# Siyou-Li/u2Tokenizer

Measured on AMD Instinct MI355X. Metric: CT volumes/sec (256^3 fp16) through u2Tokenizer fwd, higher is better.
Workload: dtype bf16; 1 GPU; BASELINE configs[2]: u2Qwen3-8B-shaped path, 256^3 volume = 8x(32,256,256) fp16, ViT-B 3D x12, SPP, 4-layer rma+diffts+dmtp tokenizer (8 heads, top_k 1024, scales {1,2,4}, 256 queries), text 1024, prompt 1024; hidden_size=4096, batch_per_gpu=1, streams_per_gpu=2, parallelism=replicas x1, tta_side_stream=off in the multi-stream run, on in the one-stream run

## Files before the change

### include/u2tok.h

```cpp
#ifndef U2TOK_H_
#define U2TOK_H_

#include <stddef.h>
#include <stdint.h>

#ifdef __cplusplus
extern "C" {
#endif

#define U2TOK_OK 0
#define U2TOK_ERR_ARG (-1)
#define U2TOK_ERR_LAUNCH (-2)
#define U2TOK_ERR_WORKSPACE (-3)
#define U2TOK_ERR_DEVICE (-4)

typedef void* u2tok_stream_t;

int u2tok_version(void);
const char* u2tok_arch(void);
const char* u2tok_elem(void);
int u2tok_device_check(void);
typedef struct u2tok_ctx* u2tok_ctx_t;
int u2tok_ctx_create(u2tok_ctx_t* out);
int u2tok_ctx_destroy(u2tok_ctx_t ctx);
int u2tok_ctx_set_current(u2tok_ctx_t ctx);
u2tok_ctx_t u2tok_ctx_get_current(void);

int u2tok_set_option(const char* name, int value);
int u2tok_set_gemm_scratch(void* device_ptr, size_t bytes, void* stream);

int u2tok_profile_collect(double* ms_host, double* flops_host, int64_t* count_host, int32_t ncat);
int u2tok_profile_collect2(double* ms_host, double* flops_host, double* bytes_host, int64_t* count_host, int32_t ncat);


typedef struct {
  int32_t nchunk;
  int32_t img[3];
  int32_t patch[3];
  int32_t hidden;
  int32_t mlp_dim;
  int32_t depth;
  int32_t heads;
  int32_t vol_dtype;
// ... 48 lines not shown
int u2tok_tokenizer_forward(const u2tok_tokenizer_config* cfg, const void* const* weights, const void* v_token,
                            const void* t_token, void* out, int64_t* topk_idx_out, void* svr_out, void* workspace,
                            size_t workspace_bytes, u2tok_stream_t stream);

typedef struct {
  const void* const* svr_in;
  void* const* svr_out;
  const void* visual_in;
  void* visual_out;
  const void* const* tta_in;
  void* const* tta_out;
} u2tok_tokenizer_taps;
int u2tok_tokenizer_forward_taps(const u2tok_tokenizer_config* cfg, const void* const* weights, const void* v_token,
                                 const void* t_token, void* out, int64_t* topk_idx_out, const u2tok_tokenizer_taps* taps,
                                 void* workspace, size_t workspace_bytes, u2tok_stream_t stream);

int u2tok_embed_splice(const void* table, const int64_t* ids, const void* feats, void* out, int32_t B, int32_t S,
                       int32_t E, int32_t nfeat, int64_t vocab, u2tok_stream_t stream);

size_t u2tok_preprocess_workspace_bytes(int32_t D, int32_t H, int32_t W);
int u2tok_preprocess_volume(const float* vol, void* out, int32_t* info, int32_t D, int32_t H, int32_t W, int32_t target,
                            int32_t depth_pad, float lower_pct, float upper_pct, int32_t out_dtype, void* workspace,
                            size_t workspace_bytes, u2tok_stream_t stream);

typedef struct {
  int32_t rot90_k;
  int32_t flip[3];
  float scale_factor;
  float shift_offset;
} u2tok_augment;
// ... 169 lines not shown
```

### u2tokenizer_amd/_lib.py

```python
from __future__ import annotations

import ctypes as C
import os
import subprocess
import threading
from pathlib import Path

_PKG = Path(__file__).resolve().parent
_LIB = _PKG / "lib" / "libu2tok_hip.so"
_LIBS = {"bf16": _LIB, "f16": _PKG / "lib" / "libu2tok_hip_f16.so"}
_lock = threading.Lock()
_handles = {}


class LibraryNotBuilt(RuntimeError):
    pass


def lib_path() -> Path:
    return _LIB


def build(verbose: bool = False) -> Path:
    cmd = ["make", "-C", str(_PKG / "csrc"), "-j", str(os.cpu_count() or 4)]
# ... 39 lines not shown
    _fields_ = [("rot90_k", C.c_int32), ("flip", C.c_int32 * 3), ("scale_factor", C.c_float), ("shift_offset", C.c_float)]


_vp, _i32, _i64, _f32, _sz = C.c_void_p, C.c_int32, C.c_int64, C.c_float, C.c_size_t

SIGNATURES = {
    "u2tok_version": (_i32, []),
    "u2tok_arch": (C.c_char_p, []),
    "u2tok_elem": (C.c_char_p, []),
    "u2tok_device_check": (_i32, []),
    "u2tok_ctx_create": (_i32, [C.POINTER(_vp)]),
    "u2tok_ctx_destroy": (_i32, [_vp]),
    "u2tok_ctx_set_current": (_i32, [_vp]),
    "u2tok_ctx_get_current": (_vp, []),
    "u2tok_set_option": (_i32, [C.c_char_p, _i32]),
    "u2tok_profile_collect": (_i32, [_vp, _vp, _vp, _i32]),
    "u2tok_profile_collect2": (_i32, [_vp, _vp, _vp, _vp, _i32]),
    "u2tok_set_gemm_scratch": (_i32, [_vp, _sz, _vp]),
    "u2tok_vit_workspace_bytes": (_sz, [C.POINTER(VitConfig)]),
    "u2tok_vit_forward": (_i32, [C.POINTER(VitConfig), C.POINTER(_vp), _vp, _vp, _vp, _sz, _vp]),
    "u2tok_spp_workspace_bytes": (_sz, [C.POINTER(SppConfig)]),
    "u2tok_spp_forward": (_i32, [C.POINTER(SppConfig), C.POINTER(_vp), _vp, _vp, _vp, _sz, _vp]),
    "u2tok_tokenizer_workspace_bytes": (_sz, [C.POINTER(TokConfig)]),
    "u2tok_tokenizer_forward": (_i32, [C.POINTER(TokConfig), C.POINTER(_vp), _vp, _vp, _vp, _vp, _vp, _vp, _sz, _vp]),
    "u2tok_tokenizer_forward_taps": (_i32, [C.POINTER(TokConfig), C.POINTER(_vp), _vp, _vp, _vp, _vp, C.POINTER(TokTaps),
                                            _vp, _sz, _vp]),
    "u2tok_tok_attention_workspace_bytes": (_sz, [_i32, _i32, _i32, _i32, _i32]),
    "u2tok_tok_attention": (_i32, [_vp, _vp, _vp, _vp, _i32, _i32, _i32, _i32, _i32, _i64, _i64, _i64, _i64, _i64, _i64, _i64,
                                   _i64, _f32, _vp, _i32, _i32, _vp, _sz, _vp]),
    "u2tok_preprocess_workspace_bytes": (_sz, [_i32, _i32, _i32]),
    "u2tok_preprocess_volume": (_i32, [_vp, _vp, _vp, _i32, _i32, _i32, _i32, _i32, _f32, _f32, _i32, _vp, _sz, _vp]),
    "u2tok_preprocess_volume_aug": (_i32, [_vp, _vp, _vp, _i32, _i32, _i32, _i32, _i32, _f32, _f32, _i32,
                                           C.POINTER(Augment), _vp, _sz, _vp]),
    "u2tok_embed_splice": (_i32, [_vp, _vp, _vp, _vp, _i32, _i32, _i32, _i32, _i64, _vp]),
    "u2tok_gemm_bf16": (_i32, [_vp, _vp, _vp, _vp, _vp, _i32, _i32, _i32, _i64, _i64, _i64, _i64, _i32, _i32,
                               _i64, _i64, _i64, _i64, _i64, _i64, _i64, _i64, _f32, _i32, _vp]),
    "u2tok_layernorm_bf16": (_i32, [_vp, _vp, _vp, _vp, _vp, _i32, _i32, _f32, _vp]),
    "u2tok_softmax_rows": (_i32, [_vp, _vp, _i32, _i32, _i32, _i64, _i64, _f32, _vp, _i32, _i32, _vp]),
    "u2tok_transpose_bf16": (_i32, [_vp, _vp, _i32, _i32, _i32, _i64, _i64, _i64, _i64, _i32, _vp]),
    "u2tok_im2col_patches": (_i32, [_vp, _i32, _vp, _i32, _i32, _i32, _i32, _i32, _i32, _i32, _vp]),
    "u2tok_avgpool3d_tokens": (_i32, [_vp, _vp, _i32, _i32, _i32, _i32, _i32, _i32, _i32, _i32, _vp]),
# ... 117 lines not shown
```

### u2tokenizer_amd/csrc/capi.hip

```cpp
#include <math.h>
#include <string.h>
#include <new>
#include "pipeline.h"

using namespace u2;

static_assert(U2TOK_OK == U2_OK && U2TOK_ERR_ARG == U2_ERR_ARG && U2TOK_ERR_LAUNCH == U2_ERR_LAUNCH &&
                  U2TOK_ERR_WORKSPACE == U2_ERR_WORKSPACE && U2TOK_ERR_DEVICE == U2_ERR_DEVICE,
              "public and internal status codes must agree");

#define BF(p) reinterpret_cast<const bf16_t*>(p)
#define BFW(p) reinterpret_cast<bf16_t*>(p)
#define ST(s) reinterpret_cast<hipStream_t>(s)

extern "C" {

int u2tok_version(void) { return 100;  }
const char* u2tok_arch(void) { return "gfx950"; }
const char* u2tok_elem(void) { return U2_ELEM_ASM; }

int u2tok_device_check(void) {
  int dev = 0;
  if (hipGetDevice(&dev) != hipSuccess) return U2_ERR_DEVICE;
  hipDeviceProp_t prop;
// ... 7 lines not shown
  return *out ? U2_OK : U2_ERR_ARG;
}
int u2tok_ctx_destroy(u2tok_ctx_t c) {
  if (!c) return U2_ERR_ARG;
  Context* cx = reinterpret_cast<Context*>(c);
  if (ctx_bound() == cx) ctx_bind(nullptr);
  delete cx;
  return U2_OK;
}
int u2tok_ctx_set_current(u2tok_ctx_t c) {
  ctx_bind(reinterpret_cast<Context*>(c));
  return U2_OK;
}
u2tok_ctx_t u2tok_ctx_get_current(void) { return reinterpret_cast<u2tok_ctx_t>(ctx_bound()); }

int u2tok_set_option(const char* name, int value) {
  if (!name) return U2_ERR_ARG;
  Options& o = ctx().opt;
  struct Opt { const char* name; int Options::*field; int lo, hi; };
  static const Opt table[] = {
      {"gemm_splitk", &Options::gemm_splitk, -1, 16},   {"gemm_mubuf", &Options::gemm_mubuf, 0, 1}, {"ln_wide", &Options::ln_wide, 0, 1},   {"gemm_big", &Options::gemm_big, -1, 27},
      {"gemm_big_grid", &Options::gemm_big_grid, 1, 4096}, {"gemm_big_splitk", &Options::gemm_big_splitk, 0, 16},
      {"gemm_big_drain", &Options::gemm_big_drain, 0, 1}, {"gemm_skinny", &Options::gemm_skinny, 0, 2},
       {"kmajor_b", &Options::kmajor_b, 0, 1},            {"gemm_tail_fused", &Options::gemm_tail_fused, 0, 1},
      {"flash_mode", &Options::flash_mode, 0, 7},        {"flash_q_prescaled", &Options::flash_q_prescaled, 0, 1},
      {"vit_flash", &Options::vit_flash, 0, 1},         {"tta_overlap", &Options::tta_overlap, 0, 1},
      {"vit_vt_epilogue", &Options::vit_vt_epilogue, 0, 1},
      {"tok_flash", &Options::tok_flash, 0, 1},
      {"tok_wide", &Options::tok_wide, 0, 2},
  };
  if (!strcmp(name, "gemm_tile")) {
    if (value != 0 && value != 64 && value != 128) return U2_ERR_ARG;
    o.gemm_tile = value;
    return U2_OK;
  }
  if (!strcmp(name, "profile")) { prof_enable(value != 0); return U2_OK; }
  for (const Opt& t : table)
    if (!strcmp(name, t.name)) {
      if (value < t.lo || value > t.hi) return U2_ERR_ARG;
      if (t.field == &Options::gemm_big && value > 0 && !(value >= 20 && value <= 27 && value != 23 && value != 25)) return U2_ERR_ARG;
      if (t.field == &Options::flash_mode && value != 0 && value != 1 && value != 7) return U2_ERR_ARG;
      o.*(t.field) = value;
      return U2_OK;
    }
  return U2_ERR_ARG;
}

int u2tok_set_gemm_scratch(void* device_ptr, size_t bytes, void* stream) {
  ctx().set_scratch(reinterpret_cast<hipStream_t>(stream), device_ptr, device_ptr ? bytes : 0);
  return U2_OK;
}

int u2tok_profile_collect(double* ms, double* flops, int64_t* count, int32_t ncat) {
  if (!ms || !flops || !count || ncat <= 0 || ncat > PROF_NCAT) return U2_ERR_ARG;
  return prof_collect(ms, flops, nullptr, count, ncat);
}
int u2tok_profile_collect2(double* ms, double* flops, double* bytes, int64_t* count, int32_t ncat) {
  if (!ms || !flops || !bytes || !count || ncat <= 0 || ncat > PROF_NCAT) return U2_ERR_ARG;
  return prof_collect(ms, flops, bytes, count, ncat);
}

// ... 30 lines not shown
  return peak + 256;
}
int u2tok_tokenizer_forward(const u2tok_tokenizer_config* cfg, const void* const* weights, const void* v_token,
                            const void* t_token, void* out, int64_t* topk_idx_out, void* svr_out, void* workspace,
                            size_t workspace_bytes, u2tok_stream_t stream) {
  if (!cfg || !workspace || ((uintptr_t)workspace & 255)) return U2_ERR_ARG;
  return tokenizer_forward(*cfg, weights, BF(v_token), BF(t_token), BFW(out), topk_idx_out, BFW(svr_out), nullptr, workspace,
                           workspace_bytes, false, nullptr, ST(stream));
}
int u2tok_tokenizer_forward_taps(const u2tok_tokenizer_config* cfg, const void* const* weights, const void* v_token,
                                 const void* t_token, void* out, int64_t* topk_idx_out, const u2tok_tokenizer_taps* taps,
                                 void* workspace, size_t workspace_bytes, u2tok_stream_t stream) {
  if (!cfg || !taps || !workspace || ((uintptr_t)workspace & 255)) return U2_ERR_ARG;
  return tokenizer_forward(*cfg, weights, BF(v_token), BF(t_token), BFW(out), topk_idx_out, nullptr, taps, workspace,
                           workspace_bytes, false, nullptr, ST(stream));
}

size_t u2tok_preprocess_workspace_bytes(int32_t D, int32_t H, int32_t W) { return preprocess_workspace_bytes(D, H, W); }
int u2tok_preprocess_volume(const float* vol, void* out, int32_t* info, int32_t D, int32_t H, int32_t W, int32_t target,
                            int32_t depth_pad, float lower_pct, float upper_pct, int32_t out_dtype, void* workspace,
                            size_t workspace_bytes, u2tok_stream_t stream) {
  return preprocess_volume(vol, out, info, D, H, W, target, depth_pad, lower_pct, upper_pct, out_dtype, nullptr, workspace,
                           workspace_bytes, ST(stream));
}
int u2tok_preprocess_volume_aug(const float* vol, void* out, int32_t* info, int32_t D, int32_t H, int32_t W, int32_t target,
                                int32_t depth_pad, float lower_pct, float upper_pct, int32_t out_dtype,
                                const u2tok_augment* aug, void* workspace, size_t workspace_bytes, u2tok_stream_t stream) {
  if (!aug) return U2_ERR_ARG;
  PreAugment a;
  a.rot_k = aug->rot90_k;
// ... 355 lines not shown
```

### u2tokenizer_amd/csrc/ctx.h

```cpp
#pragma once
#include <mutex>
#include <vector>
#include "common.h"

namespace u2 {

struct Options {
  int ln_wide = 1;
  int gemm_tile = 0;
  int gemm_mubuf = 1;
  int gemm_splitk = 0;
  int gemm_big = 0;
  int gemm_big_grid = 256;
  int gemm_big_splitk = 0;
  int gemm_big_drain = 1;
  int gemm_skinny = 2;
  int gemm_tail_fused = 1;
  int kmajor_b = 1;
  int flash_mode = 0;
  int flash_q_prescaled = 0;
  int vit_flash = 1;
  int vit_vt_epilogue = 1;
  int tok_flash = 1;
  int tok_wide = 2;
  int tta_overlap = 1;
  int profile = 0;
};

struct SideStream {
  hipStream_t owner = nullptr;
  hipStream_t s = nullptr;
  hipEvent_t fork = nullptr;
  hipEvent_t done[16] = {};
};

struct Scratch {
  hipStream_t st;
  void* p;
  size_t bytes;
};

struct ProfRec {
  hipEvent_t a, b;
  int cat;
  double flops, bytes;
};

struct Context {
  Options opt;
  std::mutex mu;
  std::vector<SideStream*> sides;
  std::vector<Scratch> scratch;
  std::vector<ProfRec> recs;
  std::vector<hipEvent_t> ev_pool;
  size_t ev_used = 0;

  SideStream* side_for(hipStream_t owner);
  void set_scratch(hipStream_t st, void* p, size_t bytes);
  Scratch scratch_of(hipStream_t st);
  void release();
  ~Context() { release(); }
};

Context& ctx();
// ... 6 lines not shown
```

### u2tokenizer_amd/csrc/pipeline.h

```cpp
#pragma once
#include <algorithm>
#include "../../include/u2tok.h"
#include "kernels.h"

namespace u2 {

typedef u2tok_vit_config VitConfig;
typedef u2tok_spp_config SppConfig;
typedef u2tok_tokenizer_config TokConfig;
typedef u2tok_tokenizer_taps TokTaps;

int vit_forward(const VitConfig& c, const void* const* W, const void* volume, bf16_t* out, void* ws, size_t ws_bytes,
                bool dry, size_t* peak, hipStream_t st);
int spp_forward(const SppConfig& c, const void* const* W, const bf16_t* x, bf16_t* out, void* ws, size_t ws_bytes,
                bool dry, size_t* peak, hipStream_t st);
int tokenizer_forward(const TokConfig& c, const void* const* W, const bf16_t* v_token, const bf16_t* t_token,
                      bf16_t* out, int64_t* topk_idx_out, bf16_t* svr_out, const TokTaps* taps, void* ws, size_t ws_bytes,
                      bool dry, size_t* peak, hipStream_t st);

}
```

### u2tokenizer_amd/csrc/pipeline.hip

```cpp
#include "pipeline.h"

namespace u2 {

namespace {

struct Arena {
  char* base;
  size_t cap;
  size_t off = 0, peak = 0;
  bool dry;
  Arena(void* b, size_t c, bool d) : base((char*)b), cap(c), dry(d) {}
  template <typename T>
  T* get(size_t count) {
    const size_t a = (off + 255) & ~(size_t)255;
    off = a + count * sizeof(T);
    if (off > peak) peak = off;
    if (dry) return reinterpret_cast<T*>((uintptr_t)0x1000 + a);
    return (off <= cap) ? reinterpret_cast<T*>(base + a) : nullptr;
  }
  bool ok() const { return dry || peak <= cap; }
};

struct ScratchScope {
  Context& cx;
// ... 275 lines not shown
  return a.wk && a.bk && a.wv == a.wk + (size_t)E * E && a.bv == a.bk + E;
}
inline bool qkv_packed(const Att& a, int E) {
  return a.wq && a.bq && a.wk == a.wq + (size_t)E * E && a.bk == a.bq + E && kv_packed(a, E);
}
int qkv_proj(const bf16_t* x, const Att& a, bf16_t* out, int64_t rows, int E, bool dry, hipStream_t st) {
  if (!dry && qkv_packed(a, E)) {
    U2_RUN(linear(x, E, a.wq, a.bq, out, 3 * E, rows, E, 3 * E, 0, nullptr, 0, st));
    return U2_OK;
  }
  U2_RUN(linear(x, E, a.wq, a.bq, out, 3 * E, rows, E, E, 0, nullptr, 0, st));
  U2_RUN(linear(x, E, a.wk, a.bk, out + E, 3 * E, rows, E, E, 0, nullptr, 0, st));
  U2_RUN(linear(x, E, a.wv, a.bv, out + 2 * E, 3 * E, rows, E, E, 0, nullptr, 0, st));
  return U2_OK;
}
}

int tokenizer_forward(const TokConfig& c, const void* const* W, const bf16_t* v_token, const bf16_t* t_token,
                      bf16_t* out, int64_t* topk_idx_out, bf16_t* svr_out, const TokTaps* taps, void* ws, size_t ws_bytes,
                      bool dry, size_t* peak, hipStream_t st) {
  if (c.B <= 0 || c.T <= 0 || c.N <= 0 || c.E <= 0 || c.Lt <= 0 || c.num_heads <= 0 || c.num_layers < 0) return U2_ERR_ARG;
  if (c.E % c.num_heads || (c.E / c.num_heads) % 8 || c.top_k <= 0 || c.num_query <= 0) return U2_ERR_ARG;
  if (c.attn_type < 0 || c.attn_type > 2) return U2_ERR_ARG;
  if (!dry && (!W || !v_token || !t_token || !out)) return U2_ERR_ARG;
  const int B = c.B, T = c.T, N = c.N, E = c.E, H = c.num_heads, d = E / H, L = c.num_layers, Q = c.num_query;
  const int TN = T * N, k = c.top_k;
  if (!c.enable_diffts && k > TN) return U2_ERR_ARG;
  if (N > c.max_seq_len || T > c.max_seq_len || Q > c.max_seq_len) return U2_ERR_ARG;
  const float scale = 1.0f / sqrtf((float)d);
  auto wp = [&](int i) { return dry ? nullptr : reinterpret_cast<const bf16_t*>(W[i]); };
  auto att_at = [&](int i) {
    Att a{wp(i), wp(i + 1), wp(i + 2), wp(i + 3), wp(i + 4), wp(i + 5), wp(i + 6), wp(i + 7), wp(i + 8)};
    if (c.attn_type != 0) a.rb = nullptr;
    return a;
  };
  const int i_sel = 1 + 18 * L, i_gate = i_sel + 2, i_tta = i_gate + 2, i_lin = i_tta + 33 * L;

  Arena ar(ws, ws_bytes, dry);
  const size_t kSplitK = std::max<size_t>(24u << 20, (size_t)16 * B * c.num_query * 3 * E);
  char* skw = ar.get<char>(kSplitK);
  U2_CHECK_WS(ar);
  Context& cx = ctx();
  ScratchScope scratch_scope(cx, st, skw, kSplitK, !dry);
  const int64_t rows = (int64_t)B * TN;
  bf16_t* xa = ar.get<bf16_t>((size_t)rows * E);
  bf16_t* xb = ar.get<bf16_t>((size_t)rows * E);
  bf16_t* qkv = ar.get<bf16_t>((size_t)rows * 3 * E);
  bf16_t* ctx = ar.get<bf16_t>((size_t)rows * E);
  U2_CHECK_WS(ar);

  const bf16_t* x = v_token;
  for (int l = 0; l < L; ++l) {
    const Att sp = att_at(1 + 18 * l), tp = att_at(1 + 18 * l + 9);
    if (taps && !dry && taps->svr_in && taps->svr_in[l]) x = reinterpret_cast<const bf16_t*>(taps->svr_in[l]);
// ... 157 lines not shown
  if (overlap && !dry) {
    if (hipEventRecord(side->fork, st) != hipSuccess || hipStreamWaitEvent(side->s, side->fork, 0) != hipSuccess)
      return U2_ERR_LAUNCH;
    for (int l = 0; l < L; ++l) {
      const int base = i_tta + 33 * l;
      Att va = att_at(base + 9), ta = att_at(base + 18);
      { const int e = kv_proj(va, V, Lv, kv_v[l], side->s); if (e != U2_OK) return e; }
      if (hipEventRecord(side->done[2 * l], side->s) != hipSuccess) return U2_ERR_LAUNCH;
      { const int e = kv_proj(ta, t_token, c.Lt, kv_t[l], side->s); if (e != U2_OK) return e; }
      if (hipEventRecord(side->done[2 * l + 1], side->s) != hipSuccess) return U2_ERR_LAUNCH;
    }
    const Att la = att_at(i_lin);
    U2_RUN(linear(V, E, la.wk, la.bk, k_lin, E, (int64_t)B * Lv, E, E, 0, nullptr, 0, side->s));
    if (hipEventRecord(side->done[2 * L], side->s) != hipSuccess) return U2_ERR_LAUNCH;
  }
  U2_RUN(fill_rows(wp(0), qa, B, (int64_t)Q * E, (int64_t)Q * E, st));
  bf16_t* qcur = qa;
  auto cross = [&](const Att& a, const bf16_t* src, int Ls, const bf16_t* qin, bf16_t* dst, bf16_t* kv,
                   int kv_ready) -> int {
    U2_RUN(linear(qin, E, a.wq, a.bq, qproj, E, qrows, E, E, 0, nullptr, 0, st));
    if (kv_ready < 0) {
      const int e = kv_proj(a, src, Ls, kv, st);
      if (e != U2_OK) return e;
    } else if (!dry) {
      if (hipStreamWaitEvent(st, side->done[kv_ready], 0) != hipSuccess) return U2_ERR_LAUNCH;
    }
    AttnCore ac{qproj, kv, kv + E, E, 2 * E, 2 * E, (int64_t)Q * E, (int64_t)Ls * 2 * E, (int64_t)Ls * 2 * E,
                qctx, E, (int64_t)Q * E, B, Q, Ls, H, d, scale, nullptr, 0};
    const int e = attention_core(ar, ac, dry, st);
    if (e != U2_OK) return e;
    U2_RUN(linear(qctx, E, a.wd, a.bd, dst, E, qrows, E, E, 0, nullptr, 0, st));
    return U2_OK;
  };
  for (int l = 0; l < L; ++l) {
    const int base = i_tta + 33 * l;
    const Att sa = att_at(base);
    Att va = att_at(base + 9), ta = att_at(base + 18);
    va.rb = ta.rb = nullptr;
    const bf16_t *ns_w = wp(base + 27), *ns_b = wp(base + 28), *nv_w = wp(base + 29), *nv_b = wp(base + 30),
                 *nt_w = wp(base + 31), *nt_b = wp(base + 32);
    if (taps && !dry && taps->tta_in && taps->tta_in[l]) qcur = (bf16_t*)taps->tta_in[l];
    bf16_t* s1 = (qcur == qa) ? qb : qa;
    bf16_t* s2 = qc;
    if (c.attn_type == 2 && B == 1) {
      U2_RUN(linear(qcur, E, sa.wv, sa.bv, qctx, E, qrows, E, E, 0, nullptr, 0, st));
    } else if (c.attn_type == 2) {
      { const int e = qkv_proj(qcur, sa, qproj, qrows, E, dry, st); if (e != U2_OK) return e; }
      const int e = chunk_axis_attention(ar, qproj, qctx, 1, B, Q, H, d, scale, nullptr, c.max_seq_len, dry, st);
      if (e != U2_OK) return e;
    } else {
      { const int e = qkv_proj(qcur, sa, qproj, qrows, E, dry, st); if (e != U2_OK) return e; }
      if (c.attn_type == 1) {
        U2_RUN(rope_apply(qproj, B, Q, 1, H, d, 3 * E, c.max_seq_len, 0, st));
        U2_RUN(rope_apply(qproj + E, B, Q, 1, H, d, 3 * E, c.max_seq_len, 0, st));
      }
      AttnCore ac{qproj, qproj + E, qproj + 2 * E, 3 * E, 3 * E, 3 * E, (int64_t)Q * 3 * E, (int64_t)Q * 3 * E,
                  (int64_t)Q * 3 * E, qctx, E, (int64_t)Q * E, B, Q, Q, H, d, scale, sa.rb, c.max_seq_len};
      const int e = attention_core(ar, ac, dry, st);
      if (e != U2_OK) return e;
    }
    U2_RUN(linear(qctx, E, sa.wd, sa.bd, qo, E, qrows, E, E, 0, nullptr, 0, st));
    U2_RUN(layernorm_bf16(qcur, qo, ns_w, ns_b, s1, 1, (int)qrows, E, 0, E, 0, E, 0, E, c.ln_eps, st));
    { const int e = cross(va, V, Lv, s1, qo, overlap ? kv_v[l] : kv_inline, overlap ? 2 * l : -1); if (e != U2_OK) return e; }
    U2_RUN(layernorm_bf16(s1, qo, nv_w, nv_b, s2, 1, (int)qrows, E, 0, E, 0, E, 0, E, c.ln_eps, st));
    { const int e = cross(ta, t_token, c.Lt, s2, qo, overlap ? kv_t[l] : kv_inline, overlap ? 2 * l + 1 : -1); if (e != U2_OK) return e; }
    U2_RUN(layernorm_bf16(s2, qo, nt_w, nt_b, s1, 1, (int)qrows, E, 0, E, 0, E, 0, E, c.ln_eps, st));
    qcur = s1;
    if (taps && !dry && taps->tta_out && taps->tta_out[l] &&
        hipMemcpyAsync(taps->tta_out[l], qcur, (size_t)qrows * E * sizeof(bf16_t), hipMemcpyDeviceToDevice, st) != hipSuccess)
      return U2_ERR_LAUNCH;
  }
  {
    const Att la = att_at(i_lin);
    U2_RUN(linear(qcur, E, la.wq, la.bq, qproj, E, qrows, E, E, 0, nullptr, 0, st));
    if (!overlap) {
      U2_RUN(linear(V, E, la.wk, la.bk, k_lin, E, (int64_t)B * Lv, E, E, 0, nullptr, 0, st));
    } else if (!dry) {
      if (hipStreamWaitEvent(st, side->done[2 * L], 0) != hipSuccess) return U2_ERR_LAUNCH;
    }
    AttnCore ac{qproj, k_lin, V, E, E, E, (int64_t)Q * E, (int64_t)Lv * E, (int64_t)Lv * E,
                out, E, (int64_t)Q * E, B, Q, Lv, H, d, scale, nullptr, 0};
    const int e = attention_core(ar, ac, dry, st);
// ... 9 lines not shown
```

### u2tokenizer_amd/tokenizer.py

```python
from __future__ import annotations

import ctypes as C

import torch
import torch.nn as nn

from . import _lib, ops

_ATTN_TYPES = {"rma": 0, "rope": 1}


def _init_attn(m):
    for lin in (m.wq, m.wk, m.wv, m.dense):
        nn.init.xavier_uniform_(lin.weight)
        if lin.bias is not None:
            nn.init.zeros_(lin.bias)


class RelativeMultiheadAttention(nn.Module):

    def __init__(self, d_model, num_heads, max_seq_len=512):
        super().__init__()
        assert d_model % num_heads == 0
        self.num_heads, self.d_model, self.depth, self.max_seq_len = num_heads, d_model, d_model // num_heads, max_seq_len
# ... 176 lines not shown
        if embed_size != hidden_size:
            raise ValueError("embed_size must equal hidden_size (builder.py:5,11 pass config.hidden_size for both)")
        self.svt_module = SpatioTemporalVisualTokenRefinerModel(
            embed_size=embed_size, num_heads=num_heads, num_layers=num_layers, top_k=top_k,
            use_multi_scale=use_multi_scale, attn_type=attn_type, enable_diffts=enable_diffts,
            enable_dmtp=enable_dmtp)
        self.tta_module = TextConditionTokenAggregatorModel(d_model=embed_size, num_layers=num_layers,
                                                            num_heads=num_heads, attn_type=attn_type)
        self.query_tokens = nn.Parameter(torch.zeros(1, num_3d_query_token, hidden_size))
        self.query_tokens.data.normal_(mean=0.0, std=0.02)
        self.embed_size, self.num_heads, self.num_layers, self.top_k = embed_size, num_heads, num_layers, top_k
        self.use_multi_scale, self.num_query, self.attn_type = bool(use_multi_scale), num_3d_query_token, attn_type
        self.enable_diffts, self.enable_dmtp = bool(enable_diffts), bool(enable_dmtp)
        self._ws = ops._Workspace()
        self._packed_key = None
        self._dead_offloaded = False
        self._register_state_dict_hook(_unshare_packed)
        self.last_topk_indices = None
        self.capture_svr_tokens = False
        self.last_svr_tokens = None

    def _weights(self):
        w = [self.query_tokens]
        for layer in self.svt_module.attention_network.layers:
            w += _att_ptrs(layer.spatial_attention) + _att_ptrs(layer.temporal_attention)
        sn = self.svt_module.token_selection.score_net
        w += [sn.weight, sn.bias]
        if self.enable_dmtp:
            w += [self.svt_module.dynamic_pool.gate_fc.weight, self.svt_module.dynamic_pool.gate_fc.bias]
        else:
# ... 10 lines not shown
        key = (self.query_tokens.data_ptr(), self.query_tokens.dtype)
        if self._packed_key == key:
            return
        with torch.no_grad():
            for layer in self.svt_module.attention_network.layers:
                _pack_qkv(layer.spatial_attention)
                _pack_qkv(layer.temporal_attention)
            for layer in self.tta_module.layers_vt:
                for m in (layer.self_attention, layer.visual_cross_attention, layer.text_cross_attention):
                    _pack_qkv(m)
        if self.query_tokens.is_cuda:
            torch.cuda.synchronize(self.query_tokens.device)
        self._packed_key = key

    def _apply(self, fn, *args, **kwargs):
        r = super()._apply(fn, *args, **kwargs)
        self._packed_key = None
        if self.query_tokens.is_cuda:
            self.pack_weights()
            if self._dead_offloaded:
                self.offload_dead_parameters()
        return r

    def dead_parameters(self):
        la = self.tta_module.layer_linagg.linear_aggregator
        return [la.wv.weight, la.wv.bias, la.dense.weight, la.dense.bias]

    def offload_dead_parameters(self) -> int:
        freed = 0
        for p in self.dead_parameters():
            if p.is_cuda:
                freed += p.numel() * p.element_size()
                p.data = p.data.to("cpu")
            p.requires_grad_(False)
        self._dead_offloaded = True
        return freed

# ... 40 lines not shown
            return arr

        svr_out = [torch.empty((B, T, N, E), dtype=ops.elem_dtype(), device=dev) for _ in range(L)]
        tta_out = [torch.empty((B, Q, E), dtype=ops.elem_dtype(), device=dev) for _ in range(L)]
        visual_out = torch.empty((B, Lv, E), dtype=ops.elem_dtype(), device=dev)
        if visual_in is not None:
            visual_in = ops._need(visual_in, ops.ELEM, "visual_in").contiguous()
            assert tuple(visual_in.shape) == (B, Lv, E)
        taps = _lib.TokTaps(svr_in=ptr_array(svr_in, (B, T, N, E)), svr_out=ptr_array(svr_out, (B, T, N, E)),
                            visual_in=None if visual_in is None else visual_in.data_ptr(), visual_out=visual_out.data_ptr(),
                            tta_in=ptr_array(tta_in, (B, Q, E)), tta_out=ptr_array(tta_out, (B, Q, E)))
        with ops.on_device(v_token) as (h, stream):
            ws = self._ws.get(nbytes, dev)
            out = torch.empty((B, Q, E), dtype=ops.elem_dtype(), device=dev)
            idx = None if self.enable_diffts else torch.empty((B, self.top_k), dtype=torch.int64, device=dev)
            _lib.check(h.u2tok_tokenizer_forward_taps(C.byref(cfg), table, v_token.data_ptr(), t_token.data_ptr(),
                                                      out.data_ptr(), None if idx is None else idx.data_ptr(),
                                                      C.byref(taps), ws.data_ptr(), ws.numel(), stream),
                       "u2tok_tokenizer_forward_taps")
        self.last_topk_indices = idx
        return out, {"svr_out": svr_out, "visual_out": visual_out, "tta_out": tta_out}

    def _config(self, B, T, N, E, Lt):
        return _lib.TokConfig(B=B, T=T, N=N, E=E, Lt=Lt, num_heads=self.num_heads,
                              num_layers=self.num_layers, top_k=self.top_k, num_query=self.num_query,
                              use_multi_scale=int(self.use_multi_scale), attn_type=_ATTN_TYPES.get(self.attn_type, 2),
                              enable_diffts=int(self.enable_diffts), enable_dmtp=int(self.enable_dmtp),
                              max_seq_len=512, diffts_tau=float(getattr(self.svt_module.token_selection, "tau", 1.0)),
                              ln_eps=1e-5)

    def forward(self, v_token, t_token):
        with ops.on_device(v_token, elem=self.query_tokens.dtype):
            return self._forward(v_token, t_token)

# ... 18 lines not shown
        self._check_envelope(B, T, N, E, t_token.shape[1])
        cfg = self._config(B, T, N, E, t_token.shape[1])
        table = ops.weight_table(self._weights())
        nbytes = h.u2tok_tokenizer_workspace_bytes(C.byref(cfg))
        if nbytes == 0:
            raise RuntimeError("u2tok_tokenizer_workspace_bytes rejected the configuration "
                               f"(B={B}, T={T}, N={N}, E={E}, heads={self.num_heads}, top_k={self.top_k})")
        idx = svr = None
        with ops.on_device(v_token) as (h, stream):
            ws = self._ws.get(nbytes, v_token.device)
            out = torch.empty((B, self.num_query, E), dtype=ops.elem_dtype(), device=v_token.device)
            if not self.enable_diffts:
                idx = torch.empty((B, self.top_k), dtype=torch.int64, device=v_token.device)
            if self.capture_svr_tokens:
                svr = torch.empty((B, T * N, E), dtype=ops.elem_dtype(), device=v_token.device)
            _lib.check(h.u2tok_tokenizer_forward(C.byref(cfg), table, v_token.data_ptr(), t_token.data_ptr(),
                                                 out.data_ptr(), None if idx is None else idx.data_ptr(),
                                                 None if svr is None else svr.data_ptr(), ws.data_ptr(), ws.numel(),
                                                 stream), "u2tok_tokenizer_forward")
        self.last_topk_indices = idx
        self.last_svr_tokens = svr
        return out
```

Measured before the change: 128.2 volumes/s.

## Precompute and cache weight-only first TTA layer query prefix across forwards

Adds a C API that computes, from weights alone, the first TTA layer's query self-attention, norm and visual-query projection. It also adds a prefixed forward entry that consumes these results in place of recomputing them. The Python tokenizer caches the prefix per batch size and invalidates it on weight version, pointer, option-epoch or context change. This removes a few small per-call GEMMs and an attention at the cost of cache management, host synchronisation when the prefix is rebuilt, and extra option plumbing.

```diff
diff --git a/include/u2tok.h b/include/u2tok.h
--- a/include/u2tok.h
+++ b/include/u2tok.h
@@ -27,6 +27,8 @@
 u2tok_ctx_t u2tok_ctx_get_current(void);
 
 int u2tok_set_option(const char* name, int value);
+int u2tok_get_option(const char* name, int* value);
+int64_t u2tok_option_epoch(void);
 int u2tok_set_gemm_scratch(void* device_ptr, size_t bytes, void* stream);
 
 int u2tok_profile_collect(double* ms_host, double* flops_host, int64_t* count_host, int32_t ncat);
@@ -105,6 +107,13 @@
 int u2tok_tokenizer_forward_taps(const u2tok_tokenizer_config* cfg, const void* const* weights, const void* v_token,
                                  const void* t_token, void* out, int64_t* topk_idx_out, const u2tok_tokenizer_taps* taps,
                                  void* workspace, size_t workspace_bytes, u2tok_stream_t stream);
+
+int u2tok_tokenizer_query_prefix(const u2tok_tokenizer_config* cfg, const void* const* weights, void* s1_out, void* q_out,
+                                 void* workspace, size_t workspace_bytes, u2tok_stream_t stream);
+int u2tok_tokenizer_forward_prefixed(const u2tok_tokenizer_config* cfg, const void* const* weights, const void* v_token,
+                                     const void* t_token, void* out, int64_t* topk_idx_out, void* svr_out,
+                                     const u2tok_tokenizer_taps* taps, const void* prefix_s1, const void* prefix_q,
+                                     void* workspace, size_t workspace_bytes, u2tok_stream_t stream);
 
 int u2tok_embed_splice(const void* table, const int64_t* ids, const void* feats, void* out, int32_t B, int32_t S,
                        int32_t E, int32_t nfeat, int64_t vocab, u2tok_stream_t stream);
diff --git a/u2tokenizer_amd/_lib.py b/u2tokenizer_amd/_lib.py
--- a/u2tokenizer_amd/_lib.py
+++ b/u2tokenizer_amd/_lib.py
@@ -77,6 +77,8 @@
     "u2tok_ctx_set_current": (_i32, [_vp]),
     "u2tok_ctx_get_current": (_vp, []),
     "u2tok_set_option": (_i32, [C.c_char_p, _i32]),
+    "u2tok_get_option": (_i32, [C.c_char_p, C.POINTER(_i32)]),
+    "u2tok_option_epoch": (_i64, []),
     "u2tok_profile_collect": (_i32, [_vp, _vp, _vp, _i32]),
     "u2tok_profile_collect2": (_i32, [_vp, _vp, _vp, _vp, _i32]),
     "u2tok_set_gemm_scratch": (_i32, [_vp, _sz, _vp]),
@@ -88,6 +90,9 @@
     "u2tok_tokenizer_forward": (_i32, [C.POINTER(TokConfig), C.POINTER(_vp), _vp, _vp, _vp, _vp, _vp, _vp, _sz, _vp]),
     "u2tok_tokenizer_forward_taps": (_i32, [C.POINTER(TokConfig), C.POINTER(_vp), _vp, _vp, _vp, _vp, C.POINTER(TokTaps),
                                             _vp, _sz, _vp]),
+    "u2tok_tokenizer_query_prefix": (_i32, [C.POINTER(TokConfig), C.POINTER(_vp), _vp, _vp, _vp, _sz, _vp]),
+    "u2tok_tokenizer_forward_prefixed": (_i32, [C.POINTER(TokConfig), C.POINTER(_vp), _vp, _vp, _vp, _vp, _vp,
+                                                C.POINTER(TokTaps), _vp, _vp, _vp, _sz, _vp]),
     "u2tok_tok_attention_workspace_bytes": (_sz, [_i32, _i32, _i32, _i32, _i32]),
     "u2tok_tok_attention": (_i32, [_vp, _vp, _vp, _vp, _i32, _i32, _i32, _i32, _i32, _i64, _i64, _i64, _i64, _i64, _i64, _i64,
                                    _i64, _f32, _vp, _i32, _i32, _vp, _sz, _vp]),
diff --git a/u2tokenizer_amd/csrc/capi.hip b/u2tokenizer_amd/csrc/capi.hip
--- a/u2tokenizer_amd/csrc/capi.hip
+++ b/u2tokenizer_amd/csrc/capi.hip
@@ -45,37 +45,51 @@
 }
 u2tok_ctx_t u2tok_ctx_get_current(void) { return reinterpret_cast<u2tok_ctx_t>(ctx_bound()); }
 
+namespace {
+struct Opt { const char* name; int Options::*field; int lo, hi; };
+const Opt kOptions[] = {
+    {"gemm_splitk", &Options::gemm_splitk, -1, 16},   {"gemm_mubuf", &Options::gemm_mubuf, 0, 1}, {"ln_wide", &Options::ln_wide, 0, 1},   {"gemm_big", &Options::gemm_big, -1, 27},
+    {"gemm_big_grid", &Options::gemm_big_grid, 1, 4096}, {"gemm_big_splitk", &Options::gemm_big_splitk, 0, 16},
+    {"gemm_big_drain", &Options::gemm_big_drain, 0, 1}, {"gemm_skinny", &Options::gemm_skinny, 0, 2},
+     {"kmajor_b", &Options::kmajor_b, 0, 1},            {"gemm_tail_fused", &Options::gemm_tail_fused, 0, 1},
+    {"flash_mode", &Options::flash_mode, 0, 7},        {"flash_q_prescaled", &Options::flash_q_prescaled, 0, 1},
+    {"vit_flash", &Options::vit_flash, 0, 1},         {"tta_overlap", &Options::tta_overlap, 0, 1},
+    {"vit_vt_epilogue", &Options::vit_vt_epilogue, 0, 1},
+    {"tok_flash", &Options::tok_flash, 0, 1},
+    {"tok_wide", &Options::tok_wide, 0, 2},
+    {"tta_prefix", &Options::tta_prefix, 0, 1},
+    {"gemm_tile", &Options::gemm_tile, 0, 128},
+};
+}
+
 int u2tok_set_option(const char* name, int value) {
   if (!name) return U2_ERR_ARG;
   Options& o = ctx().opt;
-  struct Opt { const char* name; int Options::*field; int lo, hi; };
-  static const Opt table[] = {
-      {"gemm_splitk", &Options::gemm_splitk, -1, 16},   {"gemm_mubuf", &Options::gemm_mubuf, 0, 1}, {"ln_wide", &Options::ln_wide, 0, 1},   {"gemm_big", &Options::gemm_big, -1, 27},
-      {"gemm_big_grid", &Options::gemm_big_grid, 1, 4096}, {"gemm_big_splitk", &Options::gemm_big_splitk, 0, 16},
-      {"gemm_big_drain", &Options::gemm_big_drain, 0, 1}, {"gemm_skinny", &Options::gemm_skinny, 0, 2},
-       {"kmajor_b", &Options::kmajor_b, 0, 1},            {"gemm_tail_fused", &Options::gemm_tail_fused, 0, 1},
-      {"flash_mode", &Options::flash_mode, 0, 7},        {"flash_q_prescaled", &Options::flash_q_prescaled, 0, 1},
-      {"vit_flash", &Options::vit_flash, 0, 1},         {"tta_overlap", &Options::tta_overlap, 0, 1},
-      {"vit_vt_epilogue", &Options::vit_vt_epilogue, 0, 1},
-      {"tok_flash", &Options::tok_flash, 0, 1},
-      {"tok_wide", &Options::tok_wide, 0, 2},
-  };
-  if (!strcmp(name, "gemm_tile")) {
-    if (value != 0 && value != 64 && value != 128) return U2_ERR_ARG;
-    o.gemm_tile = value;
-    return U2_OK;
-  }
   if (!strcmp(name, "profile")) { prof_enable(value != 0); return U2_OK; }
-  for (const Opt& t : table)
+  for (const Opt& t : kOptions)
     if (!strcmp(name, t.name)) {
       if (value < t.lo || value > t.hi) return U2_ERR_ARG;
+      if (t.field == &Options::gemm_tile && value != 0 && value != 64 && value != 128) return U2_ERR_ARG;
       if (t.field == &Options::gemm_big && value > 0 && !(value >= 20 && value <= 27 && value != 23 && value != 25)) return U2_ERR_ARG;
       if (t.field == &Options::flash_mode && value != 0 && value != 1 && value != 7) return U2_ERR_ARG;
+      if (o.*(t.field) != value) ++ctx().opt_epoch;
       o.*(t.field) = value;
       return U2_OK;
     }
   return U2_ERR_ARG;
 }
+
+int u2tok_get_option(const char* name, int* value) {
+  if (!name || !value) return U2_ERR_ARG;
+  for (const Opt& t : kOptions)
+    if (!strcmp(name, t.name)) {
+      *value = ctx().opt.*(t.field);
+      return U2_OK;
+    }
+  return U2_ERR_ARG;
+}
+
+int64_t u2tok_option_epoch(void) { return ctx().opt_epoch; }
 
 int u2tok_set_gemm_scratch(void* device_ptr, size_t bytes, void* stream) {
   ctx().set_scratch(reinterpret_cast<hipStream_t>(stream), device_ptr, device_ptr ? bytes : 0);
@@ -136,6 +150,21 @@
   if (!cfg || !taps || !workspace || ((uintptr_t)workspace & 255)) return U2_ERR_ARG;
   return tokenizer_forward(*cfg, weights, BF(v_token), BF(t_token), BFW(out), topk_idx_out, nullptr, taps, workspace,
                            workspace_bytes, false, nullptr, ST(stream));
+}
+int u2tok_tokenizer_query_prefix(const u2tok_tokenizer_config* cfg, const void* const* weights, void* s1_out, void* q_out,
+                                 void* workspace, size_t workspace_bytes, u2tok_stream_t stream) {
+  if (!cfg || !workspace || ((uintptr_t)workspace & 255)) return U2_ERR_ARG;
+  if (((uintptr_t)s1_out | (uintptr_t)q_out) & 255) return U2_ERR_ARG;
+  return tokenizer_query_prefix(*cfg, weights, BFW(s1_out), BFW(q_out), workspace, workspace_bytes, ST(stream));
+}
+int u2tok_tokenizer_forward_prefixed(const u2tok_tokenizer_config* cfg, const void* const* weights, const void* v_token,
+                                     const void* t_token, void* out, int64_t* topk_idx_out, void* svr_out,
+                                     const u2tok_tokenizer_taps* taps, const void* prefix_s1, const void* prefix_q,
+                                     void* workspace, size_t workspace_bytes, u2tok_stream_t stream) {
+  if (!cfg || !workspace || ((uintptr_t)workspace & 255)) return U2_ERR_ARG;
+  if (!prefix_s1 != !prefix_q || (((uintptr_t)prefix_s1 | (uintptr_t)prefix_q) & 255)) return U2_ERR_ARG;
+  return tokenizer_forward(*cfg, weights, BF(v_token), BF(t_token), BFW(out), topk_idx_out, BFW(svr_out), taps, workspace,
+                           workspace_bytes, false, nullptr, ST(stream), BF(prefix_s1), BF(prefix_q));
 }
 
 size_t u2tok_preprocess_workspace_bytes(int32_t D, int32_t H, int32_t W) { return preprocess_workspace_bytes(D, H, W); }
diff --git a/u2tokenizer_amd/csrc/ctx.h b/u2tokenizer_amd/csrc/ctx.h
--- a/u2tokenizer_amd/csrc/ctx.h
+++ b/u2tokenizer_amd/csrc/ctx.h
@@ -24,6 +24,7 @@
   int tok_flash = 1;
   int tok_wide = 2;
   int tta_overlap = 1;
+  int tta_prefix = 1;
   int profile = 0;
 };
 
@@ -48,6 +49,7 @@
 
 struct Context {
   Options opt;
+  int64_t opt_epoch = 0;
   std::mutex mu;
   std::vector<SideStream*> sides;
   std::vector<Scratch> scratch;
diff --git a/u2tokenizer_amd/csrc/pipeline.h b/u2tokenizer_amd/csrc/pipeline.h
--- a/u2tokenizer_amd/csrc/pipeline.h
+++ b/u2tokenizer_amd/csrc/pipeline.h
@@ -16,6 +16,8 @@
                 bool dry, size_t* peak, hipStream_t st);
 int tokenizer_forward(const TokConfig& c, const void* const* W, const bf16_t* v_token, const bf16_t* t_token,
                       bf16_t* out, int64_t* topk_idx_out, bf16_t* svr_out, const TokTaps* taps, void* ws, size_t ws_bytes,
-                      bool dry, size_t* peak, hipStream_t st);
+                      bool dry, size_t* peak, hipStream_t st, const bf16_t* pre_s1 = nullptr, const bf16_t* pre_q = nullptr);
+int tokenizer_query_prefix(const TokConfig& c, const void* const* W, bf16_t* s1_out, bf16_t* q_out, void* ws, size_t ws_bytes,
+                           hipStream_t st);
 
 }
diff --git a/u2tokenizer_amd/csrc/pipeline.hip b/u2tokenizer_amd/csrc/pipeline.hip
--- a/u2tokenizer_amd/csrc/pipeline.hip
+++ b/u2tokenizer_amd/csrc/pipeline.hip
@@ -313,14 +313,88 @@
   U2_RUN(linear(x, E, a.wv, a.bv, out + 2 * E, 3 * E, rows, E, E, 0, nullptr, 0, st));
   return U2_OK;
 }
+
+inline size_t tok_splitk_bytes(const TokConfig& c) {
+  return std::max<size_t>(24u << 20, (size_t)16 * c.B * c.num_query * 3 * c.E);
+}
+
+struct TtaHead {
+  Att sa, va;
+  const bf16_t *ns_w, *ns_b;
+  bf16_t *qproj, *qctx, *qo;
+};
+int tta_layer_head(const TokConfig& c, Arena& ar, const TtaHead& h, const bf16_t* qcur, bf16_t* s1, bf16_t* qv, bool dry,
+                   hipStream_t st) {
+  const int B = c.B, E = c.E, H = c.num_heads, d = E / H, Q = c.num_query;
+  const int64_t qrows = (int64_t)B * Q;
+  const float scale = 1.0f / sqrtf((float)d);
+  const Att& sa = h.sa;
+  if (c.attn_type == 2 && B == 1) {
+    U2_RUN(linear(qcur, E, sa.wv, sa.bv, h.qctx, E, qrows, E, E, 0, nullptr, 0, st));
+  } else if (c.attn_type == 2) {
+    { const int e = qkv_proj(qcur, sa, h.qproj, qrows, E, dry, st); if (e != U2_OK) return e; }
+    const int e = chunk_axis_attention(ar, h.qproj, h.qctx, 1, B, Q, H, d, scale, nullptr, c.max_seq_len, dry, st);
+    if (e != U2_OK) return e;
+  } else {
+    { const int e = qkv_proj(qcur, sa, h.qproj, qrows, E, dry, st); if (e != U2_OK) return e; }
+    if (c.attn_type == 1) {
+      U2_RUN(rope_apply(h.qproj, B, Q, 1, H, d, 3 * E, c.max_seq_len, 0, st));
+      U2_RUN(rope_apply(h.qproj + E, B, Q, 1, H, d, 3 * E, c.max_seq_len, 0, st));
+    }
+    AttnCore ac{h.qproj, h.qproj + E, h.qproj + 2 * E, 3 * E, 3 * E, 3 * E, (int64_t)Q * 3 * E, (int64_t)Q * 3 * E,
+                (int64_t)Q * 3 * E, h.qctx, E, (int64_t)Q * E, B, Q, Q, H, d, scale, sa.rb, c.max_seq_len};
+    const int e = attention_core(ar, ac, dry, st);
+    if (e != U2_OK) return e;
+  }
+  U2_RUN(linear(h.qctx, E, sa.wd, sa.bd, h.qo, E, qrows, E, E, 0, nullptr, 0, st));
+  U2_RUN(layernorm_bf16(qcur, h.qo, h.ns_w, h.ns_b, s1, 1, (int)qrows, E, 0, E, 0, E, 0, E, c.ln_eps, st));
+  U2_RUN(linear(s1, E, h.va.wq, h.va.bq, qv, E, qrows, E, E, 0, nullptr, 0, st));
+  return U2_OK;
+}
+
+inline bool tok_config_ok(const TokConfig& c) {
+  if (c.B <= 0 || c.T <= 0 || c.N <= 0 || c.E <= 0 || c.Lt <= 0 || c.num_heads <= 0 || c.num_layers < 0) return false;
+  if (c.E % c.num_heads || (c.E / c.num_heads) % 8 || c.top_k <= 0 || c.num_query <= 0) return false;
+  return c.attn_type >= 0 && c.attn_type <= 2;
+}
+}
+
+int tokenizer_query_prefix(const TokConfig& c, const void* const* W, bf16_t* s1_out, bf16_t* q_out, void* ws, size_t ws_bytes,
+                           hipStream_t st) {
+  if (!tok_config_ok(c) || c.num_layers <= 0 || c.num_query > c.max_seq_len) return U2_ERR_ARG;
+  if (!W || !s1_out || !q_out) return U2_ERR_ARG;
+  const bool dry = false;
+  const int B = c.B, E = c.E, L = c.num_layers, Q = c.num_query;
+  const int64_t qrows = (int64_t)B * Q;
+  auto wp = [&](int i) { return reinterpret_cast<const bf16_t*>(W[i]); };
+  const int base = 1 + 18 * L + 4;
+  Arena ar(ws, ws_bytes, dry);
+  const size_t kSplitK = tok_splitk_bytes(c);
+  char* skw = ar.get<char>(kSplitK);
+  bf16_t* qa = ar.get<bf16_t>((size_t)qrows * E);
+  TtaHead h;
+  h.qproj = ar.get<bf16_t>((size_t)qrows * 3 * E);
+  h.qctx = ar.get<bf16_t>((size_t)qrows * E);
+  h.qo = ar.get<bf16_t>((size_t)qrows * E);
+  U2_CHECK_WS(ar);
+  ScratchScope scratch_scope(ctx(), st, skw, kSplitK, true);
+  auto att_at = [&](int i) {
+    Att a{wp(i), wp(i + 1), wp(i + 2), wp(i + 3), wp(i + 4), wp(i + 5), wp(i + 6), wp(i + 7), wp(i + 8)};
+    if (c.attn_type != 0) a.rb = nullptr;
+    return a;
+  };
+  h.sa = att_at(base);
+  h.va = att_at(base + 9);
+  h.va.rb = nullptr;
+  h.ns_w = wp(base + 27); h.ns_b = wp(base + 28);
+  U2_RUN(fill_rows(wp(0), qa, B, (int64_t)Q * E, (int64_t)Q * E, st));
+  return tta_layer_head(c, ar, h, qa, s1_out, q_out, dry, st);
 }
 
 int tokenizer_forward(const TokConfig& c, const void* const* W, const bf16_t* v_token, const bf16_t* t_token,
                       bf16_t* out, int64_t* topk_idx_out, bf16_t* svr_out, const TokTaps* taps, void* ws, size_t ws_bytes,
-                      bool dry, size_t* peak, hipStream_t st) {
-  if (c.B <= 0 || c.T <= 0 || c.N <= 0 || c.E <= 0 || c.Lt <= 0 || c.num_heads <= 0 || c.num_layers < 0) return U2_ERR_ARG;
-  if (c.E % c.num_heads || (c.E / c.num_heads) % 8 || c.top_k <= 0 || c.num_query <= 0) return U2_ERR_ARG;
-  if (c.attn_type < 0 || c.attn_type > 2) return U2_ERR_ARG;
+                      bool dry, size_t* peak, hipStream_t st, const bf16_t* pre_s1, const bf16_t* pre_q) {
+  if (!tok_config_ok(c)) return U2_ERR_ARG;
   if (!dry && (!W || !v_token || !t_token || !out)) return U2_ERR_ARG;
   const int B = c.B, T = c.T, N = c.N, E = c.E, H = c.num_heads, d = E / H, L = c.num_layers, Q = c.num_query;
   const int TN = T * N, k = c.top_k;
@@ -336,7 +410,7 @@
   const int i_sel = 1 + 18 * L, i_gate = i_sel + 2, i_tta = i_gate + 2, i_lin = i_tta + 33 * L;
 
   Arena ar(ws, ws_bytes, dry);
-  const size_t kSplitK = std::max<size_t>(24u << 20, (size_t)16 * B * c.num_query * 3 * E);
+  const size_t kSplitK = tok_splitk_bytes(c);
   char* skw = ar.get<char>(kSplitK);
   U2_CHECK_WS(ar);
   Context& cx = ctx();
@@ -524,18 +598,22 @@
     U2_RUN(linear(V, E, la.wk, la.bk, k_lin, E, (int64_t)B * Lv, E, E, 0, nullptr, 0, side->s));
     if (hipEventRecord(side->done[2 * L], side->s) != hipSuccess) return U2_ERR_LAUNCH;
   }
-  U2_RUN(fill_rows(wp(0), qa, B, (int64_t)Q * E, (int64_t)Q * E, st));
+  const bool prefixed = !dry && pre_s1 && pre_q && L > 0 && opts().tta_prefix && !(taps && taps->tta_in && taps->tta_in[0]);
+  if (!prefixed) U2_RUN(fill_rows(wp(0), qa, B, (int64_t)Q * E, (int64_t)Q * E, st));
   bf16_t* qcur = qa;
-  auto cross = [&](const Att& a, const bf16_t* src, int Ls, const bf16_t* qin, bf16_t* dst, bf16_t* kv,
+  auto cross = [&](const Att& a, const bf16_t* src, int Ls, const bf16_t* qin, const bf16_t* qp, bf16_t* dst, bf16_t* kv,
                    int kv_ready) -> int {
-    U2_RUN(linear(qin, E, a.wq, a.bq, qproj, E, qrows, E, E, 0, nullptr, 0, st));
+    if (!qp) {
+      U2_RUN(linear(qin, E, a.wq, a.bq, qproj, E, qrows, E, E, 0, nullptr, 0, st));
+      qp = qproj;
+    }
     if (kv_ready < 0) {
       const int e = kv_proj(a, src, Ls, kv, st);
       if (e != U2_OK) return e;
     } else if (!dry) {
       if (hipStreamWaitEvent(st, side->done[kv_ready], 0) != hipSuccess) return U2_ERR_LAUNCH;
     }
-    AttnCore ac{qproj, kv, kv + E, E, 2 * E, 2 * E, (int64_t)Q * E, (int64_t)Ls * 2 * E, (int64_t)Ls * 2 * E,
+    AttnCore ac{qp, kv, kv + E, E, 2 * E, 2 * E, (int64_t)Q * E, (int64_t)Ls * 2 * E, (int64_t)Ls * 2 * E,
                 qctx, E, (int64_t)Q * E, B, Q, Ls, H, d, scale, nullptr, 0};
     const int e = attention_core(ar, ac, dry, st);
     if (e != U2_OK) return e;
@@ -550,32 +628,20 @@
     const bf16_t *ns_w = wp(base + 27), *ns_b = wp(base + 28), *nv_w = wp(base + 29), *nv_b = wp(base + 30),
                  *nt_w = wp(base + 31), *nt_b = wp(base + 32);
     if (taps && !dry && taps->tta_in && taps->tta_in[l]) qcur = (bf16_t*)taps->tta_in[l];
-    bf16_t* s1 = (qcur == qa) ? qb : qa;
+    bf16_t* nxt = (qcur == qa) ? qb : qa;
     bf16_t* s2 = qc;
-    if (c.attn_type == 2 && B == 1) {
-      U2_RUN(linear(qcur, E, sa.wv, sa.bv, qctx, E, qrows, E, E, 0, nullptr, 0, st));
-    } else if (c.attn_type == 2) {
-      { const int e = qkv_proj(qcur, sa, qproj, qrows, E, dry, st); if (e != U2_OK) return e; }
-      const int e = chunk_axis_attention(ar, qproj, qctx, 1, B, Q, H, d, scale, nullptr, c.max_seq_len, dry, st);
+    const bool pre = prefixed && l == 0;
+    const bf16_t* s1 = pre ? pre_s1 : nxt;
+    if (!pre) {
+      const TtaHead h{sa, va, ns_w, ns_b, qproj, qctx, qo};
+      const int e = tta_layer_head(c, ar, h, qcur, nxt, qproj, dry, st);
       if (e != U2_OK) return e;
-    } else {
-      { const int e = qkv_proj(qcur, sa, qproj, qrows, E, dry, st); if (e != U2_OK) return e; }
-      if (c.attn_type == 1) {
-        U2_RUN(rope_apply(qproj, B, Q, 1, H, d, 3 * E, c.max_seq_len, 0, st));
-        U2_RUN(rope_apply(qproj + E, B, Q, 1, H, d, 3 * E, c.max_seq_len, 0, st));
-      }
-      AttnCore ac{qproj, qproj + E, qproj + 2 * E, 3 * E, 3 * E, 3 * E, (int64_t)Q * 3 * E, (int64_t)Q * 3 * E,
-                  (int64_t)Q * 3 * E, qctx, E, (int64_t)Q * E, B, Q, Q, H, d, scale, sa.rb, c.max_seq_len};
-      const int e = attention_core(ar, ac, dry, st);
-      if (e != U2_OK) return e;
-    }
-    U2_RUN(linear(qctx, E, sa.wd, sa.bd, qo, E, qrows, E, E, 0, nullptr, 0, st));
-    U2_RUN(layernorm_bf16(qcur, qo, ns_w, ns_b, s1, 1, (int)qrows, E, 0, E, 0, E, 0, E, c.ln_eps, st));
-    { const int e = cross(va, V, Lv, s1, qo, overlap ? kv_v[l] : kv_inline, overlap ? 2 * l : -1); if (e != U2_OK) return e; }
+    }
+    { const int e = cross(va, V, Lv, s1, pre ? pre_q : qproj, qo, overlap ? kv_v[l] : kv_inline, overlap ? 2 * l : -1); if (e != U2_OK) return e; }
     U2_RUN(layernorm_bf16(s1, qo, nv_w, nv_b, s2, 1, (int)qrows, E, 0, E, 0, E, 0, E, c.ln_eps, st));
-    { const int e = cross(ta, t_token, c.Lt, s2, qo, overlap ? kv_t[l] : kv_inline, overlap ? 2 * l + 1 : -1); if (e != U2_OK) return e; }
-    U2_RUN(layernorm_bf16(s2, qo, nt_w, nt_b, s1, 1, (int)qrows, E, 0, E, 0, E, 0, E, c.ln_eps, st));
-    qcur = s1;
+    { const int e = cross(ta, t_token, c.Lt, s2, nullptr, qo, overlap ? kv_t[l] : kv_inline, overlap ? 2 * l + 1 : -1); if (e != U2_OK) return e; }
+    U2_RUN(layernorm_bf16(s2, qo, nt_w, nt_b, nxt, 1, (int)qrows, E, 0, E, 0, E, 0, E, c.ln_eps, st));
+    qcur = nxt;
     if (taps && !dry && taps->tta_out && taps->tta_out[l] &&
         hipMemcpyAsync(taps->tta_out[l], qcur, (size_t)qrows * E * sizeof(bf16_t), hipMemcpyDeviceToDevice, st) != hipSuccess)
       return U2_ERR_LAUNCH;
diff --git a/u2tokenizer_amd/tokenizer.py b/u2tokenizer_amd/tokenizer.py
--- a/u2tokenizer_amd/tokenizer.py
+++ b/u2tokenizer_amd/tokenizer.py
@@ -214,6 +214,8 @@
         self.enable_diffts, self.enable_dmtp = bool(enable_diffts), bool(enable_dmtp)
         self._ws = ops._Workspace()
         self._packed_key = None
+        self._prefix = {}
+        self._prefix_opt = (None, -1, False)
         self._dead_offloaded = False
         self._register_state_dict_hook(_unshare_packed)
         self.last_topk_indices = None
@@ -254,6 +256,7 @@
         self._packed_key = key
 
     def _apply(self, fn, *args, **kwargs):
+        self.invalidate_query_prefix()
         r = super()._apply(fn, *args, **kwargs)
         self._packed_key = None
         if self.query_tokens.is_cuda:
@@ -261,6 +264,47 @@
             if self._dead_offloaded:
                 self.offload_dead_parameters()
         return r
+
+    def _prefix_inputs(self):
+        layer = self.tta_module.layers_vt[0]
+        va = layer.visual_cross_attention
+        return [self.query_tokens] + [t for t in _att_ptrs(layer.self_attention) if t is not None] \
+            + [layer.norm_self.weight, layer.norm_self.bias, va.wq.weight, va.wq.bias]
+
+    def _query_prefix(self, h, cfg, table, ws, stream, device, tta_in=None):
+        if self.num_layers <= 0 or torch.is_grad_enabled() or (tta_in is not None and len(tta_in) and tta_in[0] is not None):
+            return None
+        ctxh, epoch = ops.active_context(device).handle.value, int(h.u2tok_option_epoch())
+        if self._prefix_opt[:2] != (ctxh, epoch):
+            val = C.c_int32(1)
+            _lib.check(h.u2tok_get_option(b"tta_prefix", C.byref(val)), "u2tok_get_option")
+            self._prefix_opt = (ctxh, epoch, bool(val.value))
+        if not self._prefix_opt[2] or any(p.requires_grad for p in self.parameters()):
+            return None
+        try:
+            weights = tuple((t.data_ptr(), t._version) for t in self._prefix_inputs())
+        except RuntimeError:
+            return None
+        B = int(cfg.B)
+        key = (B, ops.elem_dtype(), str(device), ctxh, epoch, weights)
+        hit = self._prefix.get(B)
+        if hit is not None and hit[0] == key:
+            return hit[1], hit[2]
+        if hit is not None:
+            torch.cuda.synchronize(device)
+            del self._prefix[B]
+        s1 = torch.empty((B, self.num_query, self.embed_size), dtype=ops.elem_dtype(), device=device)
+        q = torch.empty_like(s1)
+        _lib.check(h.u2tok_tokenizer_query_prefix(C.byref(cfg), table, s1.data_ptr(), q.data_ptr(), ws.data_ptr(), ws.numel(),
+                                                  stream), "u2tok_tokenizer_query_prefix")
+        torch.cuda.synchronize(device)
+        self._prefix[B] = (key, s1, q)
+        return s1, q
+
+    def invalidate_query_prefix(self) -> None:
+        if self._prefix and self.query_tokens.is_cuda:
+            torch.cuda.synchronize(self.query_tokens.device)
+        self._prefix = {}
 
     def dead_parameters(self):
         la = self.tta_module.layer_linagg.linear_aggregator
@@ -331,10 +375,18 @@
             ws = self._ws.get(nbytes, dev)
             out = torch.empty((B, Q, E), dtype=ops.elem_dtype(), device=dev)
             idx = None if self.enable_diffts else torch.empty((B, self.top_k), dtype=torch.int64, device=dev)
-            _lib.check(h.u2tok_tokenizer_forward_taps(C.byref(cfg), table, v_token.data_ptr(), t_token.data_ptr(),
-                                                      out.data_ptr(), None if idx is None else idx.data_ptr(),
-                                                      C.byref(taps), ws.data_ptr(), ws.numel(), stream),
-                       "u2tok_tokenizer_forward_taps")
+            pre = self._query_prefix(h, cfg, table, ws, stream, dev, tta_in)
+            if pre is not None:
+                _lib.check(h.u2tok_tokenizer_forward_prefixed(C.byref(cfg), table, v_token.data_ptr(), t_token.data_ptr(),
+                                                              out.data_ptr(), None if idx is None else idx.data_ptr(), None,
+                                                              C.byref(taps), pre[0].data_ptr(), pre[1].data_ptr(),
+                                                              ws.data_ptr(), ws.numel(), stream),
+                           "u2tok_tokenizer_forward_prefixed")
+            else:
+                _lib.check(h.u2tok_tokenizer_forward_taps(C.byref(cfg), table, v_token.data_ptr(), t_token.data_ptr(),
+                                                          out.data_ptr(), None if idx is None else idx.data_ptr(),
+                                                          C.byref(taps), ws.data_ptr(), ws.numel(), stream),
+                           "u2tok_tokenizer_forward_taps")
         self.last_topk_indices = idx
         return out, {"svr_out": svr_out, "visual_out": visual_out, "tta_out": tta_out}
 
@@ -383,10 +435,18 @@
                 idx = torch.empty((B, self.top_k), dtype=torch.int64, device=v_token.device)
             if self.capture_svr_tokens:
                 svr = torch.empty((B, T * N, E), dtype=ops.elem_dtype(), device=v_token.device)
-            _lib.check(h.u2tok_tokenizer_forward(C.byref(cfg), table, v_token.data_ptr(), t_token.data_ptr(),
-                                                 out.data_ptr(), None if idx is None else idx.data_ptr(),
-                                                 None if svr is None else svr.data_ptr(), ws.data_ptr(), ws.numel(),
-                                                 stream), "u2tok_tokenizer_forward")
+            pre = self._query_prefix(h, cfg, table, ws, stream, v_token.device)
+            if pre is not None:
+                _lib.check(h.u2tok_tokenizer_forward_prefixed(C.byref(cfg), table, v_token.data_ptr(), t_token.data_ptr(),
+                                                              out.data_ptr(), None if idx is None else idx.data_ptr(),
+                                                              None if svr is None else svr.data_ptr(), None,
+                                                              pre[0].data_ptr(), pre[1].data_ptr(), ws.data_ptr(), ws.numel(),
+                                                              stream), "u2tok_tokenizer_forward_prefixed")
+            else:
+                _lib.check(h.u2tok_tokenizer_forward(C.byref(cfg), table, v_token.data_ptr(), t_token.data_ptr(),
+                                                     out.data_ptr(), None if idx is None else idx.data_ptr(),
+                                                     None if svr is None else svr.data_ptr(), ws.data_ptr(), ws.numel(),
+                                                     stream), "u2tok_tokenizer_forward")
         self.last_topk_indices = idx
         self.last_svr_tokens = svr
         return out
```

Result: faster. 129.6 volumes/s (median of 6 runs) (+1.1%).
